# MatthewZhang473/Efficient-Gaussian-Process-on-Graphs

Hardware: NVIDIA B200
Metric: grf_walk_steps_per_sec (higher is better)
Workload: dtype f64 walk loads / f32 matvec

## Files before the change

### efficient-gaussian-process-on-graphs_b200/csrc/grf_transpose.cu

```cuda

#include "grf_common.cuh"

namespace grf {

constexpr int kRadixThreads = 256;
constexpr int kRadixWarps = kRadixThreads / 32;
constexpr int kRadixItems = 16;
constexpr int kRadixTile = kRadixThreads * kRadixItems;
constexpr int kRadixMaxBits = 10;

__global__ void __launch_bounds__(256) transpose_keys_kernel(const int32_t *__restrict__ blk_ptr,
                                                             const int2 *__restrict__ entries, int64_t n_rows,
                                                             int32_t L, int32_t entry_lo,
                                                             uint32_t *__restrict__ keys, int2 *__restrict__ payload) {
    const int lane = threadIdx.x & 31;
    const int64_t warp0 = ((int64_t)blockIdx.x * blockDim.x + threadIdx.x) >> 5;
    const int64_t nwarps = ((int64_t)gridDim.x * blockDim.x) >> 5;
    for (int64_t r = warp0; r < n_rows; r += nwarps) {
        const int32_t b = __ldg(blk_ptr + r * L), e = __ldg(blk_ptr + (r + 1) * L);
        for (int32_t i = b + lane; i < e; i += 32) {
            const int2 en = __ldg(entries + i);
            const uint32_t col = (uint32_t)en.x & kColMask, len = (uint32_t)en.x >> kStepShift;
            keys[i - entry_lo] = col * (uint32_t)L + len;
            payload[i - entry_lo] = make_int2((int32_t)((len << kStepShift) | (uint32_t)r), en.y);
        }
    }
}

__global__ void __launch_bounds__(kRadixThreads) radix_hist_kernel(const uint32_t *__restrict__ keys, int64_t n,
                                                                   int32_t shift, int32_t nbins,
                                                                   int32_t tiles_per_cta,
                                                                   int32_t *__restrict__ hist) {
    extern __shared__ uint32_t sh_hist[];
    for (int d = threadIdx.x; d < nbins; d += kRadixThreads) sh_hist[d] = 0u;
    __syncthreads();
    const uint32_t mask = (uint32_t)nbins - 1u;
    const int64_t begin = (int64_t)blockIdx.x * tiles_per_cta * kRadixTile;
    const int64_t end = min(n, begin + (int64_t)tiles_per_cta * kRadixTile);
    for (int64_t i0 = begin + threadIdx.x; i0 < end; i0 += (int64_t)kRadixThreads * 4) {
        uint32_t k[4];
#pragma unroll
        for (int u = 0; u < 4; ++u) {
            const int64_t i = i0 + (int64_t)u * kRadixThreads;
            k[u] = i < end ? __ldg(keys + i) : 0u;
        }
#pragma unroll
        for (int u = 0; u < 4; ++u) {
            const int64_t i = i0 + (int64_t)u * kRadixThreads;
            if (i < end) atomicAdd(&sh_hist[(k[u] >> shift) & mask], 1u);
        }
    }
    __syncthreads();
    for (int d = threadIdx.x; d < nbins; d += kRadixThreads) hist[(int64_t)d * gridDim.x + blockIdx.x] = (int32_t)sh_hist[d];
}

__device__ __forceinline__ uint32_t smem_u32(const void *p) { return (uint32_t)__cvta_generic_to_shared(p); }
__device__ __forceinline__ void mbar_init(uint64_t *bar, uint32_t count) {
    asm volatile("mbarrier.init.shared::cta.b64 [%1], %0;" ::"r"(count), "r"(smem_u32(bar)));
}
__device__ __forceinline__ void mbar_expect_tx(uint64_t *bar, uint32_t bytes) {
    asm volatile("mbarrier.arrive.expect_tx.shared::cta.b64 _, [%1], %0;" ::"r"(bytes), "r"(smem_u32(bar)) : "memory");
}
__device__ __forceinline__ void mbar_wait(uint64_t *bar, uint32_t parity) {
    asm volatile(
        "{\n\t"
        ".reg .pred P1;\n\t"
        "WAIT_LOOP:\n\t"
        "mbarrier.try_wait.parity.shared::cta.b64 P1, [%0], %1;\n\t"
        "@P1 bra DONE;\n\t"
        "bra WAIT_LOOP;\n\t"
        "DONE:\n\t"
        "}" ::"r"(smem_u32(bar)),
        "r"(parity)
        : "memory");
}
__device__ __forceinline__ void bulk_g2s(void *smem_dst, const void *gmem_src, uint32_t bytes, uint64_t *bar) {
    asm volatile("cp.async.bulk.shared::cluster.global.mbarrier::complete_tx::bytes [%0], [%1], %2, [%3];" ::"r"(
                     smem_u32(smem_dst)),
                 "l"(gmem_src), "r"(bytes), "r"(smem_u32(bar))
                 : "memory");
}

template <bool kLast>
__global__ void __launch_bounds__(kRadixThreads, 2) radix_scatter_kernel(const uint32_t *__restrict__ keys_in,
                                                                         const int2 *__restrict__ pay_in,
                                                                         int64_t n, int32_t shift, int32_t nbins,
                                                                         int32_t tiles_per_cta,
                                                                         const int32_t *__restrict__ offsets,
                                                                         uint32_t *__restrict__ keys_out,
                                                                         int2 *__restrict__ pay_out) {
    extern __shared__ __align__(128) unsigned char sh_bytes[];
    int2 *spay = reinterpret_cast<int2 *>(sh_bytes);
    uint32_t *skey0 = reinterpret_cast<uint32_t *>(spay + kRadixTile);
    unsigned short *xsrc = reinterpret_cast<unsigned short *>(skey0 + 2 * kRadixTile);
    uint32_t *gbase = reinterpret_cast<uint32_t *>(xsrc + kRadixTile);
    uint32_t *dstart = gbase + nbins;
    unsigned short *cnt = reinterpret_cast<unsigned short *>(dstart + nbins);
    __shared__ uint32_t warp_sums[kRadixWarps];
    __shared__ __align__(8) uint64_t bar_key[2], bar_pay;
    const int w = threadIdx.x >> 5, lane = threadIdx.x & 31;
    const uint32_t mask = (uint32_t)nbins - 1u;
    const unsigned lt = (1u << lane) - 1u;
    const int dpt = nbins >= kRadixThreads ? nbins / kRadixThreads : 1;
    const int d0 = threadIdx.x * dpt;
    const bool owner = d0 < nbins;
    const int64_t begin = (int64_t)blockIdx.x * tiles_per_cta * kRadixTile;
    const int64_t end = min(n, begin + (int64_t)tiles_per_cta * kRadixTile);
    if (begin >= end) return;
    for (int d = threadIdx.x; d < nbins; d += kRadixThreads) gbase[d] = (uint32_t)offsets[(int64_t)d * gridDim.x + blockIdx.x];
    auto key_bytes = [&](int64_t tile) { return (uint32_t)(((min((int64_t)kRadixTile, end - tile) * 4) + 15) & ~15ll); };
    auto pay_bytes = [&](int64_t tile) { return (uint32_t)(((min((int64_t)kRadixTile, end - tile) * 8) + 15) & ~15ll); };
    if (threadIdx.x == 0) {
        mbar_init(&bar_key[0], 1);
        mbar_init(&bar_key[1], 1);
        mbar_init(&bar_pay, 1);
        asm volatile("fence.mbarrier_init.release.cluster;" ::: "memory");
        mbar_expect_tx(&bar_key[0], key_bytes(begin));
        bulk_g2s(skey0, keys_in + begin, key_bytes(begin), &bar_key[0]);
        mbar_expect_tx(&bar_pay, pay_bytes(begin));
        bulk_g2s(spay, pay_in + begin, pay_bytes(begin), &bar_pay);
        if (begin + kRadixTile < end) {
            mbar_expect_tx(&bar_key[1], key_bytes(begin + kRadixTile));
            bulk_g2s(skey0 + kRadixTile, keys_in + begin + kRadixTile, key_bytes(begin + kRadixTile), &bar_key[1]);
        }
    }
    unsigned short *mycnt = cnt + w * nbins;
    uint32_t it = 0;
    for (int64_t tile = begin; tile < end; tile += kRadixTile, ++it) {
        const uint32_t *skey = skey0 + (it & 1u) * kRadixTile;
        {
            uint32_t *z = reinterpret_cast<uint32_t *>(cnt);
            for (int i = threadIdx.x; i < nbins * kRadixWarps / 2; i += kRadixThreads) z[i] = 0u;
        }
        __syncthreads();
        mbar_wait(&bar_key[it & 1u], (it >> 1) & 1u);
        const int n_tile = (int)min((int64_t)kRadixTile, end - tile);
        unsigned short rank[kRadixItems];
        const int lbase = w * (32 * kRadixItems) + lane;
#pragma unroll
        for (int k = 0; k < kRadixItems; ++k) {
            const int li = lbase + k * 32;
            const bool valid = li < n_tile;
            const uint32_t d = valid ? (skey[li] >> shift) & mask : 0u;
            const unsigned peers = __match_any_sync(0xffffffffu, valid ? d : (0x80000000u | (uint32_t)lane));
            unsigned short prev = 0;
            if (valid) prev = mycnt[d];
            __syncwarp();
            if (valid && (peers & lt) == 0u) mycnt[d] = (unsigned short)(prev + __popc(peers));
            __syncwarp();
            rank[k] = (unsigned short)(prev + __popc(peers & lt));
        }
        __syncthreads();
        uint32_t tot[4];
        uint32_t mine = 0u;
#pragma unroll
        for (int j = 0; j < 4; ++j) {
            tot[j] = 0u;
            if (j < dpt && owner) {
                const int d = d0 + j;
                uint32_t run = 0u;
#pragma unroll
                for (int ww = 0; ww < kRadixWarps; ++ww) {
                    const uint32_t c = cnt[ww * nbins + d];
                    cnt[ww * nbins + d] = (unsigned short)run;
                    run += c;
                }
                tot[j] = run;
                mine += run;
            }
        }
        uint32_t incl = mine;
#pragma unroll
        for (int dd = 1; dd < 32; dd <<= 1) {
            const uint32_t o = __shfl_up_sync(0xffffffffu, incl, dd);
            if (lane >= dd) incl += o;
        }
        if (lane == 31) warp_sums[w] = incl;
        __syncthreads();
        uint32_t before = 0u;
#pragma unroll
        for (int ww = 0; ww < kRadixWarps; ++ww) before += ww < w ? warp_sums[ww] : 0u;
        uint32_t run = before + incl - mine;
#pragma unroll
        for (int j = 0; j < 4; ++j) {
            if (j < dpt && owner) {
                dstart[d0 + j] = run;
                run += tot[j];
            }
        }
        __syncthreads();
#pragma unroll
        for (int k = 0; k < kRadixItems; ++k) {
            const int li = lbase + k * 32;
            if (li < n_tile) {
                const uint32_t d = (skey[li] >> shift) & mask;
                xsrc[dstart[d] + mycnt[d] + rank[k]] = (unsigned short)li;
            }
        }
        __syncthreads();
        mbar_wait(&bar_pay, it & 1u);
#pragma unroll 4
        for (int i = threadIdx.x; i < n_tile; i += kRadixThreads) {
            const int src = xsrc[i];
            const uint32_t kk = skey[src];
            const uint32_t d = (kk >> shift) & mask;
            const uint32_t pos = gbase[d] + ((uint32_t)i - dstart[d]);
            if (!kLast) keys_out[pos] = kk;
            pay_out[pos] = spay[src];
        }
        __syncthreads();
#pragma unroll
        for (int j = 0; j < 4; ++j)
            if (j < dpt && owner) gbase[d0 + j] += tot[j];
        if (threadIdx.x == 0) {
            const int64_t next = tile + kRadixTile, next2 = tile + 2 * (int64_t)kRadixTile;
            if (next < end) {
                mbar_expect_tx(&bar_pay, pay_bytes(next));
                bulk_g2s(spay, pay_in + next, pay_bytes(next), &bar_pay);
            }
            if (next2 < end) {
                mbar_expect_tx(&bar_key[it & 1u], key_bytes(next2));
                bulk_g2s(skey0 + (it & 1u) * kRadixTile, keys_in + next2, key_bytes(next2), &bar_key[it & 1u]);
            }
        }
    }
}

struct RadixPlan {
    int passes;
    int bits[4];
    int grid;
    int tiles_per_cta;
};

static RadixPlan radix_plan(int64_t n_keys_space, int64_t n) {
    RadixPlan p;
    const int key_bits = bit_width((uint64_t)(n_keys_space > 1 ? n_keys_space - 1 : 1));
    p.passes = (key_bits + kRadixMaxBits - 1) / kRadixMaxBits;
    if (p.passes < 1) p.passes = 1;
    const int base = key_bits / p.passes, extra = key_bits % p.passes;
    for (int i = 0; i < p.passes; ++i) p.bits[i] = base + (i >= p.passes - extra ? 1 : 0);
    for (int i = 0; i < p.passes; ++i)
        if (p.bits[i] < 1) p.bits[i] = 1;
    const int64_t tiles = (n + kRadixTile - 1) / kRadixTile;
    int64_t grid = (int64_t)kSmCount * 2;
    if (grid > tiles) grid = tiles;
    if (grid < 1) grid = 1;
    p.grid = (int)grid;
    p.tiles_per_cta = (int)((tiles + grid - 1) / grid);
    return p;
}

static inline int64_t align16(int64_t x) { return (x + 15) / 16 * 16; }

}

using namespace grf;

static int64_t transpose_counts_bytes(int64_t n_cols, int32_t n_steps) {
    return align16((n_cols * n_steps + 2) * (int64_t)sizeof(int32_t));
}

extern "C" int64_t grf_transpose_workspace_bytes(int64_t n_cols, int32_t n_steps, int64_t nnz) {
    const RadixPlan rp = radix_plan(n_cols * n_steps, nnz);
    const int64_t hist_items = (int64_t)(1 << kRadixMaxBits) * rp.grid;
    int64_t b = transpose_counts_bytes(n_cols, n_steps) + align16(grf_scan_workspace_bytes(n_cols * n_steps)) + 32;
    b += 2 * align16(nnz * 4);
    b += (rp.passes >= 2 ? 2 : 1) * align16(nnz * 8);
    b += 2 * align16((hist_items + 1) * 4) + align16(grf_scan_workspace_bytes(hist_items));
    return b;
}

namespace grf {
__global__ void __launch_bounds__(256) transpose_count_kernel(const int32_t *blk_ptr, const GrfEntry *entries,
                                                              int64_t n_rows, int32_t L, int32_t *tcnt) {
    const int lane = threadIdx.x & 31;
    const int64_t warp0 = ((int64_t)blockIdx.x * blockDim.x + threadIdx.x) >> 5;
    const int64_t nwarps = ((int64_t)gridDim.x * blockDim.x) >> 5;
    for (int64_t r = warp0; r < n_rows; r += nwarps) {
        const int32_t b = blk_ptr[r * L], e = blk_ptr[(r + 1) * L];
        for (int32_t i = b + lane; i < e; i += 32) {
            const int32_t packed = entries[i].col;
            atomicAdd(&tcnt[(int64_t)entry_col(packed) * L + entry_step(packed)], 1);
        }
    }
}
}

static inline int grid_rows(int64_t n_rows) {
    int64_t g = (n_rows + 7) / 8;
    const int64_t cap = (int64_t)kSmCount * 32;
    if (g > cap) g = cap;
    if (g < 1) g = 1;
    return (int)g;
}

extern "C" int grf_transpose_offsets(const int32_t *blk_ptr, const GrfEntry *entries, int64_t n_rows, int64_t n_cols,
                                     int32_t n_steps, const int32_t *col_counts, int32_t *tblk_ptr, void *workspace,
                                     int32_t census_threshold, int32_t *census_host, void *stream) {
    GRF_ON_STREAM_DEVICE(stream, tblk_ptr);
    GRF_REQUIRE(n_rows >= 0 && n_cols >= 0 && n_steps >= 1, "grf_transpose_offsets: bad shape");
    GRF_REQUIRE(tblk_ptr && workspace, "grf_transpose_offsets: null buffer");
    GRF_REQUIRE(!census_host || census_threshold >= 1, "grf_transpose_offsets: bad census threshold");
    cudaStream_t st = (cudaStream_t)stream;
    int32_t *tcnt = (int32_t *)workspace;
    char *scan_ws = (char *)workspace + transpose_counts_bytes(n_cols, n_steps);
    int32_t *census = (int32_t *)(scan_ws + align16(grf_scan_workspace_bytes(n_cols * n_steps)));
    if (col_counts) {
        tcnt = const_cast<int32_t *>(col_counts);
    } else if (n_cols > 0) {
        GRF_CUDA_OK(cudaMemsetAsync(tcnt, 0, (size_t)n_cols * n_steps * sizeof(int32_t), st));
        if (n_rows > 0) {
            GRF_REQUIRE(blk_ptr, "grf_transpose_offsets: null blk_ptr");
            transpose_count_kernel<<<grid_rows(n_rows), 256, 0, st>>>(blk_ptr, entries, n_rows, n_steps, tcnt);
            GRF_CUDA_OK(cudaGetLastError());
        }
    }
    int rc = grf_scan_counts(tcnt, n_cols, n_steps, GRF_ORDER_ROW_MAJOR, tblk_ptr, 0, scan_ws, stream);
    if (rc != GRF_OK) return rc;
    if (census_host) {
        rc = grf_row_census(blk_ptr, n_rows, n_steps, census_threshold, census, stream);
        if (rc != GRF_OK) return rc;
        rc = grf_row_census(tblk_ptr, n_cols, n_steps, census_threshold, census + 3, stream);
        if (rc != GRF_OK) return rc;
        GRF_CUDA_OK(cudaMemcpyAsync(census_host, census, 6 * sizeof(int32_t), cudaMemcpyDeviceToHost, st));
    }
    return GRF_OK;
}

extern "C" int grf_transpose_fill(const int32_t *blk_ptr, const GrfEntry *entries, int64_t n_rows, int64_t n_cols,
                                  int32_t n_steps, int64_t entry_lo, int64_t nnz, void *workspace,
                                  GrfEntry *tentries, void *stream) {
    GRF_ON_STREAM_DEVICE(stream, workspace);
    GRF_REQUIRE(n_rows >= 0 && n_cols >= 0 && n_steps >= 1 && nnz >= 0 && entry_lo >= 0,
                "grf_transpose_fill: bad shape");
    GRF_REQUIRE(entry_lo + nnz < (1ll << 31), "grf_transpose_fill: entry range exceeds the 32-bit offsets");
    GRF_REQUIRE(n_cols * n_steps < (1ll << 32), "grf_transpose_fill: (column, length) keys exceed 32 bits");
    if (n_cols == 0 || n_rows == 0 || nnz == 0) return GRF_OK;
    GRF_REQUIRE(blk_ptr && entries && workspace && tentries, "grf_transpose_fill: null buffer");
    cudaStream_t st = (cudaStream_t)stream;
    const RadixPlan rp = radix_plan(n_cols * n_steps, nnz);
    char *p = (char *)workspace + transpose_counts_bytes(n_cols, n_steps) +
              align16(grf_scan_workspace_bytes(n_cols * n_steps)) + 32;
    uint32_t *keys[2];
    keys[0] = (uint32_t *)p;
    p += align16(nnz * 4);
    keys[1] = (uint32_t *)p;
    p += align16(nnz * 4);
    int2 *pay[2];
    pay[0] = (int2 *)p;
    p += align16(nnz * 8);
    pay[1] = pay[0];
    if (rp.passes >= 2) {
        pay[1] = (int2 *)p;
        p += align16(nnz * 8);
    }
    const int64_t hist_cap = (int64_t)(1 << kRadixMaxBits) * rp.grid;
    int32_t *hist = (int32_t *)p;
    p += align16((hist_cap + 1) * 4);
    int32_t *offs = (int32_t *)p;
    p += align16((hist_cap + 1) * 4);
    void *scan_ws = p;

    {
        const int max_smem = kRadixTile * (8 + 2 * 4 + 2) + (1 << kRadixMaxBits) * (8 + 2 * kRadixWarps);
        GRF_CUDA_OK(cudaFuncSetAttribute(radix_scatter_kernel<true>, cudaFuncAttributeMaxDynamicSharedMemorySize, max_smem));
        GRF_CUDA_OK(cudaFuncSetAttribute(radix_scatter_kernel<false>, cudaFuncAttributeMaxDynamicSharedMemorySize, max_smem));
    }
    transpose_keys_kernel<<<grid_rows(n_rows), 256, 0, st>>>(blk_ptr, (const int2 *)entries, n_rows, n_steps,
                                                             (int32_t)entry_lo, keys[0], pay[0]);
    GRF_CUDA_OK(cudaGetLastError());
    int shift = 0;
    int cur = 0;
    for (int pass = 0; pass < rp.passes; ++pass) {
        const int nbins = 1 << rp.bits[pass];
        const bool last = pass + 1 == rp.passes;
        radix_hist_kernel<<<rp.grid, kRadixThreads, nbins * sizeof(uint32_t), st>>>(keys[cur], nnz, shift, nbins,
                                                                                     rp.tiles_per_cta, hist);
        GRF_CUDA_OK(cudaGetLastError());
        const int rc = grf_scan_counts(hist, (int64_t)nbins * rp.grid, 1, GRF_ORDER_ROW_MAJOR, offs, 0, scan_ws, stream);
        if (rc != GRF_OK) return rc;
        const size_t smem = (size_t)kRadixTile * (8 + 2 * 4 + 2) + (size_t)nbins * 2 * sizeof(uint32_t) +
                            (size_t)nbins * kRadixWarps * sizeof(unsigned short);
        if (last) {
            radix_scatter_kernel<true><<<rp.grid, kRadixThreads, smem, st>>>(
                keys[cur], pay[cur], nnz, shift, nbins, rp.tiles_per_cta, offs, nullptr, (int2 *)tentries);
        } else {
            radix_scatter_kernel<false><<<rp.grid, kRadixThreads, smem, st>>>(
                keys[cur], pay[cur], nnz, shift, nbins, rp.tiles_per_cta, offs, keys[cur ^ 1], pay[cur ^ 1]);
        }
        GRF_CUDA_OK(cudaGetLastError());
        shift += rp.bits[pass];
        cur ^= 1;
    }
    return GRF_OK;
}
```

Before: 24.43 billion.

## Fuse first radix histogram into key-building kernel with tiled row recovery

The key/payload construction kernel now works over contiguous entry tiles per CTA rather than warp-per-row. It recovers each entry's row from the block pointers through a shared-memory atomicMax marking followed by a block-wide max-scan. It also builds the first radix pass's histogram on the fly, so the separate histogram launch and its re-read of the keys are skipped for pass 0. This adds binary search, extra syncs and shared-memory scans per tile, and relies on the tiling matching radix_hist_kernel's partition.

```diff
diff --git a/efficient-gaussian-process-on-graphs_b200/csrc/grf_transpose.cu b/efficient-gaussian-process-on-graphs_b200/csrc/grf_transpose.cu
--- a/efficient-gaussian-process-on-graphs_b200/csrc/grf_transpose.cu
+++ b/efficient-gaussian-process-on-graphs_b200/csrc/grf_transpose.cu
@@ -9,22 +9,92 @@
 constexpr int kRadixTile = kRadixThreads * kRadixItems;
 constexpr int kRadixMaxBits = 10;
 
-__global__ void __launch_bounds__(256) transpose_keys_kernel(const int32_t *__restrict__ blk_ptr,
-                                                             const int2 *__restrict__ entries, int64_t n_rows,
-                                                             int32_t L, int32_t entry_lo,
-                                                             uint32_t *__restrict__ keys, int2 *__restrict__ payload) {
-    const int lane = threadIdx.x & 31;
-    const int64_t warp0 = ((int64_t)blockIdx.x * blockDim.x + threadIdx.x) >> 5;
-    const int64_t nwarps = ((int64_t)gridDim.x * blockDim.x) >> 5;
-    for (int64_t r = warp0; r < n_rows; r += nwarps) {
-        const int32_t b = __ldg(blk_ptr + r * L), e = __ldg(blk_ptr + (r + 1) * L);
-        for (int32_t i = b + lane; i < e; i += 32) {
-            const int2 en = __ldg(entries + i);
-            const uint32_t col = (uint32_t)en.x & kColMask, len = (uint32_t)en.x >> kStepShift;
-            keys[i - entry_lo] = col * (uint32_t)L + len;
-            payload[i - entry_lo] = make_int2((int32_t)((len << kStepShift) | (uint32_t)r), en.y);
-        }
-    }
+__global__ void __launch_bounds__(kRadixThreads) transpose_keys_kernel(const int32_t *__restrict__ blk_ptr,
+                                                                       const int2 *__restrict__ entries,
+                                                                       int64_t n_rows, int32_t L, int32_t entry_lo,
+                                                                       int64_t n, int64_t span, int32_t nbins,
+                                                                       uint32_t *__restrict__ keys,
+                                                                       int2 *__restrict__ payload,
+                                                                       int32_t *__restrict__ hist) {
+    extern __shared__ __align__(16) int32_t sh_keys[];
+    int32_t *row_of = sh_keys;
+    uint32_t *sh_hist = reinterpret_cast<uint32_t *>(sh_keys + kRadixTile);
+    __shared__ int32_t warp_max[kRadixWarps];
+    __shared__ int32_t sh_row;
+    const int w = threadIdx.x >> 5, lane = threadIdx.x & 31;
+    for (int d = threadIdx.x; d < nbins; d += kRadixThreads) sh_hist[d] = 0u;
+    const int64_t p0 = (int64_t)blockIdx.x * span, p1 = min(n, p0 + span);
+    if (threadIdx.x == 0 && p0 < p1) {
+        int64_t lo = 0, hi = n_rows - 1;
+        while (lo < hi) {
+            const int64_t mid = (lo + hi + 1) >> 1;
+            if ((int64_t)__ldg(blk_ptr + mid * L) - entry_lo <= p0) lo = mid; else hi = mid - 1;
+        }
+        sh_row = (int32_t)lo;
+    }
+    __syncthreads();
+    const uint32_t mask = (uint32_t)nbins - 1u;
+    int32_t r_cur = p0 < p1 ? sh_row : 0;
+    for (int64_t t0 = p0; t0 < p1; t0 += kRadixTile) {
+        const int n_tile = (int)min((int64_t)kRadixTile, p1 - t0);
+        for (int j = threadIdx.x; j < kRadixTile; j += kRadixThreads) row_of[j] = j == 0 ? r_cur : -1;
+        __syncthreads();
+        for (int64_t r = (int64_t)r_cur + 1 + threadIdx.x;; r += kRadixThreads) {
+            const int64_t start = r < n_rows ? (int64_t)__ldg(blk_ptr + r * L) - entry_lo : n;
+            const bool inside = start < t0 + n_tile;
+            if (inside) atomicMax(&row_of[start - t0], (int32_t)r);
+            if (!__syncthreads_or(threadIdx.x == kRadixThreads - 1 && inside)) break;
+        }
+        __syncthreads();
+        int4 *mine = reinterpret_cast<int4 *>(row_of + threadIdx.x * kRadixItems);
+        int32_t v[kRadixItems];
+#pragma unroll
+        for (int q = 0; q < kRadixItems / 4; ++q) {
+            const int4 x = mine[q];
+            v[4 * q] = x.x, v[4 * q + 1] = x.y, v[4 * q + 2] = x.z, v[4 * q + 3] = x.w;
+        }
+#pragma unroll
+        for (int k = 1; k < kRadixItems; ++k) v[k] = max(v[k], v[k - 1]);
+        int32_t incl = v[kRadixItems - 1];
+#pragma unroll
+        for (int dd = 1; dd < 32; dd <<= 1) {
+            const int32_t o = __shfl_up_sync(0xffffffffu, incl, dd);
+            if (lane >= dd) incl = max(incl, o);
+        }
+        if (lane == 31) warp_max[w] = incl;
+        int32_t before = __shfl_up_sync(0xffffffffu, incl, 1);
+        if (lane == 0) before = -1;
+        __syncthreads();
+#pragma unroll
+        for (int ww = 0; ww < kRadixWarps; ++ww)
+            if (ww < w) before = max(before, warp_max[ww]);
+#pragma unroll
+        for (int q = 0; q < kRadixItems / 4; ++q)
+            mine[q] = make_int4(max(v[4 * q], before), max(v[4 * q + 1], before), max(v[4 * q + 2], before),
+                                max(v[4 * q + 3], before));
+        __syncthreads();
+        r_cur = row_of[n_tile - 1];
+        int2 en[kRadixItems];
+#pragma unroll
+        for (int k = 0; k < kRadixItems; ++k) {
+            const int j = threadIdx.x + k * kRadixThreads;
+            en[k] = j < n_tile ? __ldg(entries + entry_lo + t0 + j) : make_int2(0, 0);
+        }
+#pragma unroll
+        for (int k = 0; k < kRadixItems; ++k) {
+            const int j = threadIdx.x + k * kRadixThreads;
+            if (j < n_tile) {
+                const uint32_t col = (uint32_t)en[k].x & kColMask, len = (uint32_t)en[k].x >> kStepShift;
+                const uint32_t key = col * (uint32_t)L + len;
+                keys[t0 + j] = key;
+                payload[t0 + j] = make_int2((int32_t)((len << kStepShift) | (uint32_t)row_of[j]), en[k].y);
+                atomicAdd(&sh_hist[key & mask], 1u);
+            }
+        }
+        __syncthreads();
+    }
+    __syncthreads();
+    for (int d = threadIdx.x; d < nbins; d += kRadixThreads) hist[(int64_t)d * gridDim.x + blockIdx.x] = (int32_t)sh_hist[d];
 }
 
 __global__ void __launch_bounds__(kRadixThreads) radix_hist_kernel(const uint32_t *__restrict__ keys, int64_t n,
@@ -367,17 +437,20 @@
         GRF_CUDA_OK(cudaFuncSetAttribute(radix_scatter_kernel<true>, cudaFuncAttributeMaxDynamicSharedMemorySize, max_smem));
         GRF_CUDA_OK(cudaFuncSetAttribute(radix_scatter_kernel<false>, cudaFuncAttributeMaxDynamicSharedMemorySize, max_smem));
     }
-    transpose_keys_kernel<<<grid_rows(n_rows), 256, 0, st>>>(blk_ptr, (const int2 *)entries, n_rows, n_steps,
-                                                             (int32_t)entry_lo, keys[0], pay[0]);
+    transpose_keys_kernel<<<rp.grid, kRadixThreads, kRadixTile * sizeof(int32_t) + (1 << rp.bits[0]) * sizeof(uint32_t),
+                            st>>>(blk_ptr, (const int2 *)entries, n_rows, n_steps, (int32_t)entry_lo, nnz,
+                                  (int64_t)rp.tiles_per_cta * kRadixTile, 1 << rp.bits[0], keys[0], pay[0], hist);
     GRF_CUDA_OK(cudaGetLastError());
     int shift = 0;
     int cur = 0;
     for (int pass = 0; pass < rp.passes; ++pass) {
         const int nbins = 1 << rp.bits[pass];
         const bool last = pass + 1 == rp.passes;
-        radix_hist_kernel<<<rp.grid, kRadixThreads, nbins * sizeof(uint32_t), st>>>(keys[cur], nnz, shift, nbins,
-                                                                                     rp.tiles_per_cta, hist);
-        GRF_CUDA_OK(cudaGetLastError());
+        if (pass > 0) {
+            radix_hist_kernel<<<rp.grid, kRadixThreads, nbins * sizeof(uint32_t), st>>>(keys[cur], nnz, shift, nbins,
+                                                                                         rp.tiles_per_cta, hist);
+            GRF_CUDA_OK(cudaGetLastError());
+        }
         const int rc = grf_scan_counts(hist, (int64_t)nbins * rp.grid, 1, GRF_ORDER_ROW_MAJOR, offs, 0, scan_ws, stream);
         if (rc != GRF_OK) return rc;
         const size_t smem = (size_t)kRadixTile * (8 + 2 * 4 + 2) + (size_t)nbins * 2 * sizeof(uint32_t) +
diff --git a/profiles/prof_transpose.py b/profiles/prof_transpose.py
--- /dev/null
+++ b/profiles/prof_transpose.py
@@ -0,0 +1,74 @@
+import argparse
+import json
+import os
+import subprocess
+import sys
+
+ROOT = os.path.dirname(os.path.dirname(os.path.abspath(__file__)))
+sys.path[:0] = [ROOT, os.path.join(ROOT, "efficient-gaussian-process-on-graphs_b200")]
+import torch
+
+import bench
+from grf_b200 import engine
+
+
+def main():
+    ap = argparse.ArgumentParser()
+    ap.add_argument("--out", required=True)
+    ap.add_argument("--runs", type=int, default=10)
+    args = ap.parse_args()
+    os.makedirs(args.out, exist_ok=True)
+    dev = torch.device("cuda:0")
+    gpu = subprocess.run(["nvidia-smi", "-i", "0", "--query-gpu=name,power.limit,clocks.max.sm",
+                          "--format=csv,noheader"], capture_output=True, text=True).stdout.strip()
+    graph, _ = bench.cfg4_walk_graph(bench.RMAT_SCALE, bench.RMAT_EDGES, dev)
+    cfg = engine.WalkConfig(bench.W, bench.P_HALT, bench.L, seed=bench.SEED)
+    graph.edge_records(bench.P_HALT)
+    phi = engine.build_phi_blocks(graph, cfg, transpose=False)
+    del graph
+    torch.cuda.synchronize(dev)
+    flush = torch.empty(256 << 20, dtype=torch.uint8, device=dev)
+    stream = torch.cuda.current_stream(dev)
+
+    def build():
+        phi.tblocks = None
+        phi.build_transpose()
+
+    times = []
+    for i in range(args.runs + 2):
+        phi.tblocks = None
+        torch.cuda.synchronize(dev)
+        flush.fill_(1)
+        a, b = torch.cuda.Event(enable_timing=True), torch.cuda.Event(enable_timing=True)
+        a.record(stream)
+        build()
+        b.record(stream)
+        torch.cuda.synchronize(dev)
+        if i >= 2:
+            times.append(a.elapsed_time(b))
+    ts = sorted(times)
+
+    phi.tblocks = None
+    torch.cuda.synchronize(dev)
+    with torch.profiler.profile(activities=[torch.profiler.ProfilerActivity.CUDA]) as prof:
+        build()
+        torch.cuda.synchronize(dev)
+    kernels = {}
+    for e in prof.key_averages():
+        if e.device_time_total > 0:
+            kernels[e.key] = {"calls": e.count, "total_ms": e.device_time_total / 1e3}
+    res = {
+        "what": "build_transpose() of the config-4 Phi (R-MAT 2^22, W = 100, L = 5), L2 flushed before each build",
+        "gpu": gpu, "nnz": int(phi.nnz), "n_rows": int(phi.n_rows), "n_cols": int(phi.n_cols),
+        "build_ms": {"runs": times, "median": ts[len(ts) // 2], "min": ts[0], "max": ts[-1]},
+        "kernels_one_build": dict(sorted(kernels.items(), key=lambda kv: -kv[1]["total_ms"])),
+    }
+    with open(os.path.join(args.out, "transpose.json"), "w") as fh:
+        json.dump(res, fh, indent=1)
+    print(json.dumps({"gpu": gpu, "build_ms": res["build_ms"]}))
+    for k, v in list(res["kernels_one_build"].items())[:14]:
+        print(f"{v['total_ms']:9.3f} ms  x{v['calls']:<3d} {k[:110]}")
+
+
+if __name__ == "__main__":
+    main()
```

After: 24.93 billion (median of 6 runs). +2.0%, better.
